# Bebra777228/PolGen-RVC

Measured on AMD Instinct MI355X. Metric: real-time-factor (audio-sec/wall-sec) per GPU, 30s@16kHz RMVPE->48kHz, higher is better.
Workload: dtype f32 (conv products as 3 fp16 MFMAs of a hi/lo split, fp32 accumulate; fp32 elsewhere)

## Files before the change

### polgen-rvc_amd/csrc/conv.h

```cpp
#pragma once
#include "common.h"

namespace rvcx {

enum Act { ACT_NONE = 0, ACT_LRELU = 1, ACT_RELU = 2, ACT_GELU = 3, ACT_TANH = 4, ACT_SIGMOID = 5 };
enum OutMode { OUT_NORMAL = 0, OUT_SHUF1D = 1, OUT_SHUF2D = 2, OUT_TRANSPOSED = 3 };
enum Acc2 { ACC2_NONE = 0, ACC2_SET = 1, ACC2_ADD = 2, ACC2_ADD_DIV = 3 };

struct ConvArgs {
  const float* x = nullptr;
  const float* w = nullptr;
  const void* w_h3 = nullptr;
  const void* x_split = nullptr;
  void* y_split = nullptr;
  const float* bias = nullptr;
  const float* res = nullptr;
  float* y = nullptr;
  float* y2 = nullptr;
  const int* lens_in = nullptr;
  const int* lens_out = nullptr;
  int B = 1;
  int Cin_g = 0, Cin_gp = 0, Cout_g = 0, Cout_gp = 0, groups = 1;
  int Tin = 0;
  int Nout = 0;
  int ksize = 1, kw = 1, rowpitch = 0, dil = 1, pad = 0, stride = 1;
  long x_bs = 0, y_bs = 0, res_bs = 0, y2_bs = 0;
  int x_cs = 0, y_cs = 0, res_cs = 0, y2_cs = 0;
  int pre_act = ACT_NONE;
  float pre_slope = 0.f;
  int act = ACT_NONE;
  float act_slope = 0.f;
  int out_mode = OUT_NORMAL;
  int sh_s = 1, sh_pad = 0, sh_cout = 0, sh_tout = 0;
  int wp_in = 0, wp_out = 0;
  int zero_wp = 0;
  int acc2_mode = ACC2_NONE;
  float acc2_div = 1.f;
  const float* nz_har = nullptr;
  const float* nz_w = nullptr;
  const float* nz_b = nullptr;
  const int* nz_lens = nullptr;
  int nz_k = 0, nz_stride = 1, nz_pad = 0, nz_wstride = 0;
  long nz_bs = 0;
  int nz_len = 0;
  float* part = nullptr;
  long part_cap = 0;
  long part_cap_item = 0;
  int ci_chunk = 0, kk_chunk = 0, wrow = 0, off_min = 0;
  int splitk = 1;
  long long* trace = nullptr;
  int stagger = 0;
  int stagger_blocks = 0;
  int* ovf = nullptr;
  int* ovf_layer = nullptr;
  int seq = 0;
  int dbg = 0;
};

inline int conv_tap_off(const ConvArgs& a, int kk) {
  return (kk / a.kw) * a.rowpitch + (kk % a.kw) * a.dil - a.pad;
}

struct PairArgs {
  const float* x = nullptr;
  float* y = nullptr;
  float* y2 = nullptr;
  const void* w1 = nullptr;
  const void* w2 = nullptr;
  const float* b1 = nullptr;
  const float* b2 = nullptr;
// ... 106 lines not shown
```

### polgen-rvc_amd/csrc/conv.hip

```cpp
#include "conv.h"
#include "conv_device.h"
#include "gemm.h"

#include <algorithm>
#include <cmath>

namespace rvcx {

template <int BM, int BN, int WR, int WC>
__global__ __launch_bounds__(256) void conv_mfma_kernel(const ConvArgs a) {
  constexpr int WM = BM / (32 * WR), WN = BN / (32 * WC);
  static_assert(WR * WC == 4 && WM >= 1 && WN >= 1, "bad tile");
  extern __shared__ float smem[];
  float* As = smem;
  float* Bs = smem + a.kk_chunk * a.ci_chunk * BM;

  const int tid = threadIdx.x, lane = tid & 63, wave = tid >> 6;
  const int wr = wave / WC, wc = wave % WC;
  const int i = lane & 31, h = lane >> 5;
  const int b = blockIdx.z;
  const int mt_per_g = (a.Cout_gp + BM - 1) / BM;
  const int g = blockIdx.y / mt_per_g, mt = blockIdx.y % mt_per_g;
  const int co0 = mt * BM;
  const int n0 = blockIdx.x * BN;
// ... 207 lines not shown
    return;
  }
  ProfRec rec;
  RVCX_HIP(hipEventCreate(&rec.a));
  RVCX_HIP(hipEventCreate(&rec.b));
  rec.tile = kBlock3Slot;
  rec.flops = flops;
  rec.cin = a.C; rec.cout = a.C; rec.k = 3; rec.nout = a.T; rec.stride = 135; rec.B = a.B;
  RVCX_HIP(hipEventRecord(rec.a, stream));
  launch_resblock3(a, stream);
  RVCX_HIP(hipEventRecord(rec.b, stream));
  g_prof.push_back(rec);
}

void conv_launch_gemm(const GemmArgs& a, double flops, hipStream_t stream) {
  if (!g_prof_on) {
    launch_gemm(a, stream);
    return;
  }
  ProfRec rec;
  RVCX_HIP(hipEventCreate(&rec.a));
  RVCX_HIP(hipEventCreate(&rec.b));
  rec.flops = flops;
  rec.cin = a.cin; rec.cout = a.cout; rec.k = 1; rec.nout = (int)a.rows; rec.stride = 1; rec.B = (int)(a.rows / a.T);
  RVCX_HIP(hipEventRecord(rec.a, stream));
  rec.tile = launch_gemm(a, stream);
  RVCX_HIP(hipEventRecord(rec.b, stream));
  g_prof.push_back(rec);
}

void launch_conv(ConvArgs a, hipStream_t stream) {
  RVCX_CHECK(a.Cin_gp % 2 == 0 && a.Cout_gp % 32 == 0, "conv: unpadded weights");
  RVCX_CHECK(a.Nout > 0 && a.B > 0, "conv: empty problem");
  if (g_prof_on) {
    ProfRec rec;
    RVCX_HIP(hipEventCreate(&rec.a));
    RVCX_HIP(hipEventCreate(&rec.b));
    rec.tile = 0;
    rec.flops = conv_flops(a);
    rec.cin = a.Cin_g * a.groups; rec.cout = a.Cout_g * a.groups; rec.k = a.ksize; rec.nout = a.Nout;
    rec.stride = a.stride; rec.B = a.B;
    RVCX_HIP(hipEventRecord(rec.a, stream));
    const int slot = launch_conv_fast(a, stream);
    if (slot >= 0) {
      rec.tile = slot;
      RVCX_HIP(hipEventRecord(rec.b, stream));
      g_prof.push_back(rec);
      return;
    }
    (void)hipEventDestroy(rec.a);
    (void)hipEventDestroy(rec.b);
  } else if (launch_conv_fast(a, stream) >= 0) {
    return;
  }
  int best = -1;
  double best_t = 1e300;
  ConvArgs best_a = a;
  for (int t = 0; t < kNumTiles; ++t) {
    ConvArgs c = a;
    if (!plan_lds(c, kTiles[t].bm, kTiles[t].bn)) continue;
    long mt = cdiv(a.Cout_gp, kTiles[t].bm), nt = cdiv(a.Nout, kTiles[t].bn);
    long blocks = mt * nt * a.groups;
    long rounds = (blocks + 511) / 512;
    double tm = (double)rounds * kTiles[t].bm * kTiles[t].bn / kTiles[t].eff;
    if (tm < best_t) {
      best_t = tm;
// ... 68 lines not shown
```

### polgen-rvc_amd/csrc/conv3_thin.hip

```cpp
#include <algorithm>
#include <cstdlib>
#include <mutex>

#include "conv.h"
#include "conv_device.h"
#include "h3_device.h"

namespace rvcx {

namespace {

constexpr int kTileN = 30;

__device__ __forceinline__ half8 shl1(half8 v) {
  uint4 u = __builtin_bit_cast(uint4, v);
#if defined(__HIP_DEVICE_COMPILE__)
  u.x = (unsigned)__builtin_amdgcn_update_dpp(0, (int)u.x, 0x130, 0xf, 0xf, false);
  u.y = (unsigned)__builtin_amdgcn_update_dpp(0, (int)u.y, 0x130, 0xf, 0xf, false);
  u.z = (unsigned)__builtin_amdgcn_update_dpp(0, (int)u.z, 0x130, 0xf, 0xf, false);
  u.w = (unsigned)__builtin_amdgcn_update_dpp(0, (int)u.w, 0x130, 0xf, 0xf, false);
#endif
  return __builtin_bit_cast(half8, u);
}

// ... 99 lines not shown
    }
    if (i < kTileN) {
      const int nn = p0 + i;
      if (a.y_split) store_tile_split(a, b, 0, nn, h, acc, len_out);
      else store_tile_fast(a, b, 4 * h, nn, acc, len_out);
    }
  }
  if (ovf) report_h3_overflow(a.ovf, a.ovf_layer, a.seq);
}

size_t lds_bytes(int cin) { return (size_t)(cin / 16) * 9 * 2 * 64 * 16; }

template <int CIN, bool XS>
void set_attr() {
  RVCX_HIP(hipFuncSetAttribute(reinterpret_cast<const void*>(conv3_thin_kernel<CIN, XS>),
                               hipFuncAttributeMaxDynamicSharedMemorySize, (int)lds_bytes(CIN)));
}

template <int CIN, bool XS>
void launch(const ConvArgs& a, dim3 grid, hipStream_t stream) {
  hipLaunchKernelGGL((conv3_thin_kernel<CIN, XS>), grid, dim3(256), lds_bytes(CIN), stream, a);
}

}

bool conv3_thin_ok(const ConvArgs& a) {
  static const bool on = !getenv("RVCX_CONV3_THIN") || atoi(getenv("RVCX_CONV3_THIN")) != 0;
  static const int min_n = getenv("RVCX_CONV3_THIN_MIN") ? atoi(getenv("RVCX_CONV3_THIN_MIN")) : 20000;
  if (!on || !a.w_h3 || !conv_h3_enabled() || g_conv_override.tile >= 0 || g_conv_override.splitk > 0) return false;
  if (a.groups != 1 || a.stride != 1 || a.dil != 1 || a.ksize != 9 || a.kw != 3 || a.rowpitch < 3 || a.pad != a.rowpitch + 1)
    return false;
  if (!(a.Cin_g == 16 || a.Cin_g == 32) || a.Cin_gp != a.Cin_g || a.Cout_g > 32 || a.Cout_gp > 32 || a.Cout_g < 1) return false;
  if (a.out_mode != OUT_NORMAL || a.act > ACT_RELU || a.pre_act != ACT_NONE || a.nz_har) return false;
  if (a.y_split && (a.Cout_g % 16 != 0 || a.acc2_mode != ACC2_NONE || a.res)) return false;
  if (!a.y_split && !a.y && a.acc2_mode == ACC2_NONE) return false;
  if ((long)a.Nout < min_n) return false;
  if ((long)a.Cin_g * a.x_cs * 4 >= kH3Oob || (long)a.Cout_g * a.y_cs * 4 >= kH3Oob) return false;
  return true;
}

void launch_conv3_thin(const ConvArgs& a, hipStream_t stream) {
  static std::mutex mu;
  static uint64_t done = 0;
  int dev = 0;
  RVCX_HIP(hipGetDevice(&dev));
  {
    std::lock_guard<std::mutex> g(mu);
    if (!((done >> (dev & 63)) & 1)) {
      set_attr<16, false>();
      set_attr<16, true>();
      set_attr<32, false>();
      set_attr<32, true>();
      done |= 1ull << (dev & 63);
    }
  }
  static const int ncu = [] {
    int d = 0, n = 256;
    if (hipGetDevice(&d) == hipSuccess) (void)hipDeviceGetAttribute(&n, hipDeviceAttributeMultiprocessorCount, d);
    return std::max(8, n);
  }();
  static const int per_cu_env = getenv("RVCX_CONV3_THIN_WGS") ? atoi(getenv("RVCX_CONV3_THIN_WGS")) : 0;
  const int per_cu = per_cu_env > 0 ? per_cu_env : (a.Cin_g == 16 ? 6 : 4);
  const int ntiles = cdiv(a.Nout, kTileN);
  const int per_xcd = cdiv(ntiles, 8), max_wg_x = std::max(1, ncu * per_cu / 8);
  const int rounds = cdiv(per_xcd, 4 * max_wg_x);
  const int wgs = 8 * std::max(1, cdiv(per_xcd, 4 * rounds));
// ... 14 lines not shown
```

### polgen-rvc_amd/csrc/conv_device.h

```cpp
#pragma once
#include "conv.h"

namespace rvcx {

typedef float f32x16 __attribute__((ext_vector_type(16)));

__device__ __forceinline__ void report_h3_overflow(int* ovf, int* layer, int seq) {
  if (ovf) atomicOr(ovf, kErrH3Overflow);
  if (layer) atomicMax(layer, 0x7fffffff - seq);
}

__device__ __forceinline__ float apply_act(float v, int act, float slope) {
  switch (act) {
    case ACT_LRELU: return v > 0.f ? v : v * slope;
    case ACT_RELU: return v > 0.f ? v : 0.f;
    case ACT_GELU: return 0.5f * v * (1.f + erff(v * 0.70710678118654752440f));
    case ACT_TANH: return tanhf(v);
    case ACT_SIGMOID: return 1.f / (1.f + __expf(-v));
    default: return v;
  }
}


__device__ __forceinline__ float noise_conv_at(const ConvArgs& a, int b, int c, int t) {
  const int nz_len = a.nz_lens ? a.nz_lens[b] : a.nz_len;
  const float* hb = a.nz_har + (long)b * a.nz_bs;
  const long p0 = (long)t * a.nz_stride - a.nz_pad;
  float n = 0.f;
  for (int j = 0; j < a.nz_k; ++j) {
    const long p = p0 + j;
    const float hvv = (p >= 0 && p < nz_len) ? hb[p] : 0.f;
    n = fmaf(a.nz_w[(long)j * a.nz_wstride + c], hvv, n);
  }
  return n + (a.nz_b ? a.nz_b[c] : 0.f);
}

__device__ __forceinline__ void store_elem(const ConvArgs& a, int b, int cg, int nn, float v, int len_out) {
  if (a.bias) v += a.bias[cg];
  v = apply_act(v, a.act, a.act_slope);
  if (a.out_mode == OUT_NORMAL) {
    if (a.res) v += a.res[(long)b * a.res_bs + (long)cg * a.res_cs + nn];
    if (nn >= len_out) v = 0.f;
    if (a.zero_wp > 0) {
      const int col = nn % a.zero_wp;
      if (col == 0 || col == a.zero_wp - 1) v = 0.f;
    }
    if (a.y) a.y[(long)b * a.y_bs + (long)cg * a.y_cs + nn] = v;
    if (a.acc2_mode != ACC2_NONE) {
      float* p2 = a.y2 + (long)b * a.y2_bs + (long)cg * a.y2_cs + nn;
      if (a.acc2_mode == ACC2_SET) *p2 = v;
      else if (a.acc2_mode == ACC2_ADD) *p2 = *p2 + v;
      else *p2 = (*p2 + v) / a.acc2_div;
    }
  } else if (a.out_mode == OUT_SHUF1D) {
    const int c = cg / a.sh_s, ph = cg - c * a.sh_s;
    const int t = nn * a.sh_s + ph - a.sh_pad;
    if (t >= 0 && t < a.sh_tout) {
      if (a.res) v += a.res[(long)b * a.res_bs + (long)c * a.res_cs + t];
      if (a.nz_har) v += noise_conv_at(a, b, c, t);
      if (t >= len_out) v = 0.f;
      a.y[(long)b * a.y_bs + (long)c * a.y_cs + t] = v;
    }
  } else if (a.out_mode == OUT_SHUF2D) {
    const int ph = cg / a.sh_cout, c = cg - ph * a.sh_cout;
    const int pa = ph >> 1, pb = ph & 1;
    const int irow = nn / a.wp_in, jj = nn - irow * a.wp_in;
    if (nn >= len_out) v = 0.f;
    if (jj != 0 && jj != a.wp_in - 1) {
      const long rowbase = (long)b * a.y_bs + (long)c * a.y_cs + (long)(2 * irow + pa) * a.wp_out;
      a.y[rowbase + 2 * (jj - 1) + pb + 1] = v;
      if (jj == 1 && pb == 0) a.y[rowbase] = 0.f;
      if (jj == a.wp_in - 2 && pb == 1) a.y[rowbase + a.wp_out - 1] = 0.f;
    }
  } else {
    if (a.res) v += a.res[(long)b * a.res_bs + (long)nn * a.res_cs + cg];
    if (nn >= len_out) v = 0.f;
    a.y[(long)b * a.y_bs + (long)nn * a.y_cs + cg] = v;
  }
}

__device__ __forceinline__ void store_tile(const ConvArgs& a, int b, int g, int co_base, int nn, const f32x16& t,
                                           int len_out) {
  if (nn >= a.Nout) return;
#pragma unroll
  for (int r = 0; r < 16; ++r) {
    const int co = co_base + (r & 3) + 8 * (r >> 2);
    if (co < a.Cout_g) store_elem(a, b, g * a.Cout_g + co, nn, t[r], len_out);
  }
}

__device__ __forceinline__ bool fast_epilogue_ok(const ConvArgs& a) {
  return a.out_mode == OUT_NORMAL && a.act <= ACT_RELU;
}

__device__ __forceinline__ void store_tile_fast(const ConvArgs& a, int b, int co_base, int nn, const f32x16& t,
                                                int len_out) {
  if (nn >= a.Nout) return;
  const float slope = a.act == ACT_NONE ? 1.f : (a.act == ACT_RELU ? 0.f : a.act_slope);
  bool live = nn < len_out;
  if (a.zero_wp > 0) {
    const int col = nn % a.zero_wp;
    live = live && col != 0 && col != a.zero_wp - 1;
  }
  float* yb = a.y ? a.y + (long)b * a.y_bs + nn : nullptr;
  const float* rb = a.res ? a.res + (long)b * a.res_bs + nn : nullptr;
  float* y2b = a.acc2_mode != ACC2_NONE ? a.y2 + (long)b * a.y2_bs + nn : nullptr;
#pragma unroll
  for (int r0 = 0; r0 < 16; r0 += 8) {
    float bv[8], rv[8];
#pragma unroll
    for (int q = 0; q < 8; ++q) {
      const int r = r0 + q;
      const int co = co_base + (r & 3) + 8 * (r >> 2);
      const int cc = co < a.Cout_g ? co : 0;
      bv[q] = a.bias ? a.bias[cc] : 0.f;
      rv[q] = rb ? rb[cc * a.res_cs] : 0.f;
    }
    if (y2b) {
      float pv[8];
#pragma unroll
      for (int q = 0; q < 8; ++q) {
        const int r = r0 + q;
        const int co = co_base + (r & 3) + 8 * (r >> 2);
        const int cc = co < a.Cout_g ? co : 0;
        pv[q] = a.acc2_mode != ACC2_SET ? y2b[cc * a.y2_cs] : 0.f;
// ... 71 lines not shown
```

### polgen-rvc_amd/csrc/conv_h3.hip

```cpp
#include <algorithm>
#include <cmath>
#include <cstdlib>

#include "conv.h"
#include "conv_device.h"
#include "h3_device.h"

#ifdef RVCX_ABLATION
#define H3_DBG(a, bit) ((a).dbg & (bit))
#else
#define H3_DBG(a, bit) 0
#endif

namespace rvcx {

template <int BM, int BN, int WR, int WC, int KKT, int HALO, int STRIDE, bool LIN, bool XS = false>
__global__ __launch_bounds__(256, ((LIN && BM * BN >= 8192) || BN >= 512) ? 2 : 3) void conv_h3_kernel(const ConvArgs a) {
  constexpr int WM = BM / (32 * WR), WN = BN / (32 * WC);
  constexpr int WROW = LIN ? BN : BN * STRIDE + HALO;
  constexpr int NBTILE = LIN ? KKT : 1;
  constexpr int A_ELEMS = KKT * 2 * 2 * BM;
  constexpr int NA = (A_ELEMS + 255) / 256;
  constexpr int B_TASKS = NBTILE * 2 * WROW;
  constexpr int NBT = (B_TASKS + 255) / 256;
  static_assert(WR * WC == 4, "bad tile");
  __shared__ uint4 As[A_ELEMS];
  __shared__ uint4 Bs[NBTILE * 2 * 2 * WROW];

  const int tid = threadIdx.x, lane = tid & 63, wave = tid >> 6;
  const int wr = wave / WC, wc = wave % WC;
  const int i = lane & 31, h = lane >> 5;
  const int bz = blockIdx.z / a.splitk, ks = blockIdx.z - bz * a.splitk;
  const int b = bz / a.groups, grp = bz - b * a.groups;
  const int co0 = blockIdx.y * BM;
  const int n0 = blockIdx.x * BN;
  const int len_in = a.lens_in ? a.lens_in[b] : a.Tin;
  const int in_base = n0 * STRIDE + a.off_min;
  const int wuse = LIN ? BN : BN * STRIDE + a.wrow;
  const int pre_act = a.pre_act;
  const float pre_slope = a.pre_slope;
  const int nchunk = a.Cin_gp / 16;
  constexpr bool xsplit = XS;
  static_assert(!XS || !LIN, "pre-split input: tap tiles only");
  const H3Rsrc xr = xsplit ? h3_rsrc(static_cast<const char*>(a.x_split) + (long)b * a.x_bs * 4, a.Cin_g * a.x_cs * 4)
                           : h3_rsrc(a.x + (long)b * a.x_bs + (long)grp * a.Cin_g * a.x_cs, a.Cin_g * a.x_cs * 4);
  const H3Rsrc wr_ = h3_rsrc(static_cast<const char*>(a.w_h3) + (long)grp * a.ksize * nchunk * 4 * a.Cout_gp * 16,
                             a.ksize * nchunk * 4 * a.Cout_gp * 16);

  f32x16 acc[WM][WN];
// ... 173 lines not shown
    }
    kk0 = kk1;
    chunk = chunk1;
  }

  if (ovf) report_h3_overflow(a.ovf, a.ovf_layer, a.seq);
  constexpr float inv = 1.f / kH3Scale;
#pragma unroll
  for (int m = 0; m < WM; ++m)
#pragma unroll
    for (int n = 0; n < WN; ++n)
#pragma unroll
      for (int r = 0; r < 16; ++r) acc[m][n][r] *= inv;

  const int co_w = co0 + wr * (WM * 32) + 4 * h, nn_w = n0 + wc * (WN * 32) + i;
  if (H3_DBG(a, 8)) return;
  if (a.splitk > 1) {
    float* pb = a.part + ((long)ks * a.B + b) * a.Cout_g * a.Nout;
#pragma unroll
    for (int m = 0; m < WM; ++m)
#pragma unroll
      for (int n = 0; n < WN; ++n) {
        const int nn = nn_w + n * 32;
        if (nn < a.Nout) {
#pragma unroll
          for (int r = 0; r < 16; ++r) {
            const int co = co_w + m * 32 + (r & 3) + 8 * (r >> 2);
            if (co < a.Cout_g) pb[(long)co * a.Nout + nn] = acc[m][n][r];
          }
        }
      }
    return;
  }
  if (a.y_split) {
    const int c_t = co0 + wr * (WM * 32);
#pragma unroll
    for (int m = 0; m < WM; ++m)
#pragma unroll
      for (int n = 0; n < WN; ++n) store_tile_split(a, b, c_t + m * 32, nn_w + n * 32, h, acc[m][n], len_out);
  } else if (fast_epilogue_ok(a) && a.groups == 1) {
#pragma unroll
    for (int m = 0; m < WM; ++m)
#pragma unroll
      for (int n = 0; n < WN; ++n) store_tile_fast(a, b, co_w + m * 32, nn_w + n * 32, acc[m][n], len_out);
  } else if (a.out_mode == OUT_SHUF1D) {
#pragma unroll
    for (int m = 0; m < WM; ++m)
#pragma unroll
      for (int n = 0; n < WN; ++n) store_tile_shuf1d(a, b, co_w + m * 32, nn_w + n * 32, acc[m][n], len_out);
  } else {
#pragma unroll
    for (int m = 0; m < WM; ++m)
#pragma unroll
      for (int n = 0; n < WN; ++n) store_tile(a, b, grp, co_w + m * 32, nn_w + n * 32, acc[m][n], len_out);
  }
}

namespace {
struct H3Cfg {
  int bm, bn, halo, stride;
  bool lin;
  float ovh;
  float eff;
  void (*kern)(const ConvArgs);
  void (*kern_xs)(const ConvArgs);
};
const H3Cfg kH3[] = {
    {32, 256, 64, 1, false, 18.f, 0.40f, conv_h3_kernel<32, 256, 1, 4, 4, 64, 1, false>, conv_h3_kernel<32, 256, 1, 4, 4, 64, 1, false, true>},
    {64, 128, 64, 1, false, 16.f, 0.45f, conv_h3_kernel<64, 128, 2, 2, 2, 64, 1, false>, conv_h3_kernel<64, 128, 2, 2, 2, 64, 1, false, true>},
    {64, 64, 64, 1, false, 16.f, 0.75f, conv_h3_kernel<64, 64, 2, 2, 4, 64, 1, false>, conv_h3_kernel<64, 64, 2, 2, 4, 64, 1, false, true>},
    {32, 128, 320, 1, false, 22.f, 1.00f, conv_h3_kernel<32, 128, 1, 4, 4, 320, 1, false>, conv_h3_kernel<32, 128, 1, 4, 4, 320, 1, false, true>},
    {64, 64, 320, 1, false, 20.f, 0.80f, conv_h3_kernel<64, 64, 2, 2, 4, 320, 1, false>, conv_h3_kernel<64, 64, 2, 2, 4, 320, 1, false, true>},
    {64, 128, 64, 2, false, 18.f, 0.50f, conv_h3_kernel<64, 128, 2, 2, 2, 64, 2, false>, conv_h3_kernel<64, 128, 2, 2, 2, 64, 2, false, true>},
    {64, 64, 64, 2, false, 16.f, 0.80f, conv_h3_kernel<64, 64, 2, 2, 4, 64, 2, false>, conv_h3_kernel<64, 64, 2, 2, 4, 64, 2, false, true>},
    {64, 64, 0, 1, true, 16.f, 0.95f, conv_h3_kernel<64, 64, 2, 2, 4, 0, 1, true>, nullptr},
    {128, 64, 0, 1, true, 18.f, 1.00f, conv_h3_kernel<128, 64, 4, 1, 2, 0, 1, true>, nullptr},
    {32, 256, 320, 1, false, 22.f, 1.10f, conv_h3_kernel<32, 256, 1, 4, 4, 320, 1, false>, conv_h3_kernel<32, 256, 1, 4, 4, 320, 1, false, true>},
    {32, 512, 320, 1, false, 22.f, 1.15f, conv_h3_kernel<32, 512, 1, 4, 4, 320, 1, false>, conv_h3_kernel<32, 512, 1, 4, 4, 320, 1, false, true>},
};
constexpr int kNumH3 = sizeof(kH3) / sizeof(kH3[0]);
constexpr int h3_slot(int t) { return t < 11 ? 39 + t : 28 + (t - 11); }
static_assert(kNumH3 <= 22, "conv_h3: out of profile slots");
}

thread_local bool g_force_fp32 = false;
thread_local bool g_gru_no_cluster = false;
thread_local int g_gru_drop_member = 0;

bool conv_h3_enabled() {
  static const int mode = getenv("RVCX_H3") ? atoi(getenv("RVCX_H3")) : 1;
  return mode != 0 && !g_force_fp32;
}

bool conv_h3_configured() {
  const bool saved = g_force_fp32;
  g_force_fp32 = false;
  const bool r = conv_h3_enabled();
  g_force_fp32 = saved;
  return r;
}

void conv_h3_describe(ConvProfile* p) {
  for (int t = 0; t < kNumH3; ++t) {
    const int s = h3_slot(t);
    p->bm[s] = kH3[t].bm;
    p->bn[s] = kH3[t].bn;
    p->halo[s] = 400000 + (kH3[t].lin ? 1 : (kH3[t].stride == 2 ? 2 : kH3[t].halo));
  }
}

bool conv_h3_split_ok(const ConvArgs& a) {
  if (!a.w_h3 || !conv_h3_enabled()) return false;
  if (a.groups != 1 || a.ksize == 1 || a.out_mode != OUT_NORMAL) return false;
  if (a.stride != 1 && !(a.stride == 2 && a.kw == a.ksize)) return false;
  if (a.Cin_g % 16 != 0 || a.Cout_g % 16 != 0 || a.Cin_g != a.Cin_gp) return false;
  {
    int lo = 1 << 30, hi = -(1 << 30);
    for (int kk = 0; kk < a.ksize; ++kk) {
      lo = std::min(lo, conv_tap_off(a, kk));
      hi = std::max(hi, conv_tap_off(a, kk));
    }
    if (hi - lo > 320) return false;
  }
  if ((long)a.Cin_gp * a.x_cs * 4 >= kH3Oob || (long)a.Cout_g * a.y_cs * 4 >= kH3Oob) return false;
  return true;
}

int launch_conv_h3(ConvArgs& a, int halo, int off_min, hipStream_t stream) {
  const bool split = a.x_split || a.y_split;
  RVCX_CHECK(!split || conv_h3_split_ok(a), "conv_h3: pre-split activations on a launch that cannot take them");
  if (!a.w_h3 || !conv_h3_enabled()) return -1;
  if (a.Cin_gp % 16 != 0 || (a.stride != 1 && !(a.stride == 2 && a.kw == a.ksize))) return -1;
  if (a.groups != 1 && (split || a.ksize == 1 || a.stride != 1 || a.out_mode != OUT_NORMAL || a.Cin_g != a.Cin_gp)) return -1;
  if ((long)a.Cin_gp * a.x_cs * 4 >= kH3Oob || (long)a.ksize * a.Cin_gp * a.Cout_gp * 4 >= kH3Oob) return -1;
  const bool lin = a.ksize == 1 && a.stride == 1;
  const int nchunk = a.Cin_gp / 16;
  const long cap_item = a.part_cap_item > 0 ? a.part_cap_item : a.part_cap;
  static const bool wide3x3 = getenv("RVCX_WIDE3X3") && atoi(getenv("RVCX_WIDE3X3")) != 0;
  auto select = [&](int Bsel, int forcedS, int* tile_out, int* s_out) {
    int best = -1, S = 1;
    double best_t = 1e300;
    for (int t = 0; t < kNumH3; ++t) {
      const H3Cfg& F = kH3[t];
      if (g_conv_override.tile >= 100 && g_conv_override.tile - 100 != t) continue;
      if (F.lin != lin || F.stride != a.stride) continue;
      if (a.x_split && !F.kern_xs) continue;
      if (!wide3x3 && g_conv_override.tile < 100 && F.halo == 320 && F.bn >= 256) continue;
      if (!lin && (halo > F.halo || (F.halo == 320 && halo <= 64))) continue;
      const long blocks = (long)cdiv(a.Cout_gp, F.bm) * cdiv(a.Nout, F.bn) * Bsel * a.groups;
      const double ksteps = (double)a.ksize * nchunk;
      for (int s = 1; s <= ((split || a.groups != 1) ? 1 : 8); s *= 2) {
        if (s > 1 && (!a.part || nchunk / s < 1 || ksteps / s < 8.0 || (long)s * a.Cout_g * a.Nout > cap_item ||
                      (long)s * a.B * a.Cout_g * a.Nout > a.part_cap))
          break;
        if (g_conv_override.splitk > 0 && g_conv_override.splitk != s) continue;
        if (forcedS > 0 && s != forcedS) continue;
        const double c = (double)blocks * s / 256.0;
        const double f = std::min(1.0, 0.45 + 0.55 * (std::max(c, 1.0) - 1.0) / 3.0);
        double us = std::ceil(c) * (F.bm / 32) * (F.bn / 32) * (ksteps / s + F.ovh) / (39.0 * F.eff * f);
        if (s > 1) us += 3.0 + (double)(s + 1) * Bsel * a.Cout_g * a.Nout * 4.0 / 3e6;
        if (us < best_t) {
          best_t = us;
          best = t;
          S = s;
        }
      }
    }
    *tile_out = best;
    *s_out = S;
  };
  int best = -1, S = 1;
  select(1, 0, &best, &S);
  static const int tile2_mask = getenv("RVCX_TILE2_MASK") ? atoi(getenv("RVCX_TILE2_MASK")) : 255;
  const int cls = (a.out_mode != OUT_NORMAL) ? 8 : (lin ? 2 : (halo > 64 ? 1 : 4));
  int cls2 = cls;
  if (a.x_split || a.y_split) cls2 |= 16;
  const bool tile_for_batch = (tile2_mask & cls) && (!(cls2 & 16) || (tile2_mask & 16));
  if (best >= 0 && a.B > 1 && tile_for_batch) {
    int b2 = -1, s2 = 1;
    select(a.B, S, &b2, &s2);
    if (b2 >= 0 && s2 == S) best = b2;
  }
  if (best < 0) return -1;
  const H3Cfg& F = kH3[best];
  a.off_min = off_min;
  a.wrow = halo;
  a.splitk = S;
  {
    static int dbg = -1;
    if (dbg < 0) dbg = getenv("RVCX_CONV_DBG") ? atoi(getenv("RVCX_CONV_DBG")) : 0;
    a.dbg = dbg;
  }
  dim3 grid(cdiv(a.Nout, F.bn), cdiv(a.Cout_gp, F.bm), a.B * a.groups * S);
  {
    static const bool log = getenv("RVCX_CONV_LOG") != nullptr;
    if (log)
      fprintf(stderr, "h3 tile %d (%dx%d halo %d) S %d grid %u %u %u B %d Cin %d Cout %d k %d Nout %d xs %d ys %d\n", best,
              F.bm, F.bn, F.halo, S, grid.x, grid.y, grid.z, a.B, a.Cin_g, a.Cout_g, a.ksize, a.Nout, a.x_split != nullptr,
              a.y_split != nullptr);
  }
  hipLaunchKernelGGL(a.x_split ? F.kern_xs : F.kern, grid, dim3(256), 0, stream, a);
  if (S > 1) launch_splitk_finish(a, stream);
  RVCX_HIP(hipGetLastError());
  return h3_slot(best);
}

}
```

### polgen-rvc_amd/csrc/models.h

```cpp
#pragma once
#include <functional>

#include "../../include/rvcx.h"
#include "ctx.h"
#include "layers.h"

namespace rvcx {

struct SynthModel {
  std::shared_ptr<WeightRegion> region = std::make_shared<WeightRegion>();
  rvcx_synth_cfg cfg{};
  int upp = 1;
  int dec_rf_frames = 0;
  ConvW emb_phone;
  const float* emb_pitch = nullptr;
  struct EncLayer {
    ConvW qkv, o, ffn1, ffn2;
    AttFlag att;
    const float *rel_k = nullptr, *rel_v = nullptr;
    const float *g1 = nullptr, *b1 = nullptr, *g2 = nullptr, *b2 = nullptr;
  };
  std::vector<EncLayer> enc;
  ConvW proj;
  struct Flow {
    ConvW pre, post, cond, in_l[3], rs_l[3];
  };
  Flow flows[4];
  ConvW conv_pre, cond, conv_post;
  const float* lin_wb = nullptr;
  struct Stage {
    ConvT1dW up;
    ConvW noise;
    int noise_stride = 1, noise_pad = 0;
    ConvW noise_dense;
    int noise_dense_cin = 0;
    int ch = 0;
    ConvW c1[4][3], c2[4][3];
  };
  std::vector<Stage> stages;
  const float* emb_g = nullptr;
};

std::unique_ptr<SynthModel> synth_load(Ctx& c, const rvcx_synth_cfg& cfg, const TensorTable& t);

struct SynthIO {
  int B = 1, T = 0;
  const int* lens_host = nullptr;
  const float* phone_ct = nullptr;
  const int* pitch = nullptr;
  const float* pitchf = nullptr;
  const int* sid_host = nullptr;
  const float* z_noise = nullptr;
  const float* src_noise = nullptr;
  float* out = nullptr;
  int dec_skip = 0;
  int skip_head = 0;
  float* stats_out = nullptr;
  float* z_out = nullptr;
  hipEvent_t ev_decoder = nullptr;
};
size_t synth_arena_bytes(const SynthModel& m, int B, int T);
void synth_forward(Ctx& c, const SynthModel& m, const SynthIO& io, hipEvent_t* stage_ev );

struct RmvpeModel {
  std::shared_ptr<WeightRegion> region = std::make_shared<WeightRegion>();
  rvcx_rmvpe_cfg cfg{};
  ConvW stft;
  ConvW melfb;
  const float* bn0 = nullptr;
  struct Block {
    ConvW c1, c2, sc;
    bool has_sc = false;
    int cin = 0, cout = 0;
  };
// ... 130 lines not shown
```

### polgen-rvc_amd/csrc/synth.hip

```cpp
#include <algorithm>
#include <cmath>
#include <cstdlib>

#include "models.h"
#include "ops.h"

namespace rvcx {

std::vector<float> wn_weight(const TensorTable& t, const std::string& p, int dim) {
  if (t.has(p + ".weight")) return t.f32(p + ".weight");
  std::string gn = p + ".parametrizations.weight.original0", vn = p + ".parametrizations.weight.original1";
  if (!t.has(gn)) {
    gn = p + ".weight_g";
    vn = p + ".weight_v";
  }
  std::vector<float> g = t.f32(gn), v = t.f32(vn);
  const auto shp = t.shape(vn);
  RVCX_CHECK(shp.size() == 3, "weight-norm tensor must be 3-D: " + p);
  const int64_t d0 = shp[0], d1 = shp[1], d2 = shp[2];
  std::vector<float> w(v.size());
  if (dim == 0) {
    RVCX_CHECK((int64_t)g.size() == d0, "weight_g shape: " + p);
    for (int64_t a = 0; a < d0; ++a) {
      double ss = 0.0;
// ... 143 lines not shown
size_t synth_arena_bytes(const SynthModel& m, int B, int T) {
  const auto& cf = m.cfg;
  size_t enc = (size_t)B * T * (size_t)(cf.input_dim + 8 * cf.hidden_channels + 2 * cf.filter_channels +
                                        4 * cf.inter_channels + 64 + (8 * 98 + 2 * 96 + 8) * cf.n_heads);
  size_t dec = (size_t)B * T * m.upp * 5;
  size_t mx = 0, sum = (size_t)B * T * cf.up_initial_channel;
  long tt = T;
  for (size_t i = 0; i < m.stages.size(); ++i) {
    tt *= cf.up_rates[i];
    const size_t n = (size_t)B * tt * m.stages[i].ch;
    mx = std::max(mx, n);
    sum += n + 1024;
  }
  return (enc + dec + 2 * sum + 9 * mx) * sizeof(float) + ((size_t)64 << 20);
}

namespace {

struct Timer3 {
  Ctx& c;
  hipEvent_t* e;
  Timer3(Ctx& cc, hipEvent_t* ev) : c(cc), e(ev) {}
  void mark(int i) {
    if (e) RVCX_HIP(hipEventRecord(e[i], c.stream));
  }
};

int* upload_ints(Ctx& c, const std::vector<int>& v) {
  int* d = c.arena.alloc<int>(v.size());
  RVCX_HIP(hipMemcpyAsync(d, v.data(), v.size() * sizeof(int), hipMemcpyHostToDevice, c.stream));
  return d;
}

}

void synth_forward(Ctx& c, const SynthModel& m, const SynthIO& io, hipEvent_t* stage_ev) {
  const auto& cf = m.cfg;
  const int B = io.B, T = io.T, hid = cf.hidden_channels, inter = cf.inter_channels, filt = cf.filter_channels;
  const int heads = cf.n_heads, kc = hid / heads, half = inter / 2, gin = cf.gin_channels;
  hipStream_t s = c.stream;
  Arena& A = c.arena;
  Timer3 tm(c, stage_ev);
  tm.mark(0);
  const int head = io.skip_head, Tk = T - head;
  RVCX_CHECK(head >= 0 && Tk > 0, "synth: skip_head outside [0, T)");
  if (head > 0) {
    RVCX_CHECK(io.dec_skip == 0, "synth: dec_skip and skip_head exclude each other");
    if (io.lens_host)
      for (int b = 0; b < B; ++b) RVCX_CHECK(io.lens_host[b] == T, "synth: skip_head needs equal lengths (every item T frames)");
  }

  bool ragged = false;
  if (io.lens_host)
    for (int b = 0; b < B; ++b) ragged |= io.lens_host[b] != T;
  std::vector<const int*> lens_stage(m.stages.size() + 2, nullptr);
  const int* lens = nullptr;
  if (ragged) {
    std::vector<int> l(io.lens_host, io.lens_host + B);
    lens = upload_ints(c, l);
    lens_stage[0] = lens;
    for (size_t i = 0; i < m.stages.size(); ++i) {
      for (auto& x : l) x *= cf.up_rates[i];
      lens_stage[i + 1] = upload_ints(c, l);
    }
  }
  std::vector<int> sidv(io.sid_host, io.sid_host + B);
// ... 78 lines not shown
    a.lens_out = lens;
    conv_set_res(a, x, hid, T);
    c.conv(a);
    launch_layernorm_c(tmp, L.g1, L.b1, x, B, hid, T, 1e-5f, nullptr, s);
    const int k = L.ffn1.k, pl = (k - 1) / 2;
    a = conv1d_args(L.ffn1, x, hbuf, B, T, T, 1, 1, pl);
    a.act = ACT_RELU;
    a.lens_in = lens;
    a.lens_out = lens;
    c.conv(a);
    a = conv1d_args(L.ffn2, hbuf, tmp, B, T, T, 1, 1, pl);
    a.lens_in = lens;
    a.lens_out = lens;
    conv_set_res(a, x, hid, T);
    c.conv(a);
    launch_layernorm_c(tmp, L.g2, L.b2, x, B, hid, T, 1e-5f, nullptr, s);
  }
  float* stats = io.stats_out ? io.stats_out : A.alloc<float>((size_t)B * 2 * inter * T);
  {
    launch_mask(x, B, hid, T, lens, s);
    ConvArgs a = conv1d_args(m.proj, x, stats, B, T, T);
    a.lens_out = lens;
    c.conv(a);
  }
  tm.mark(1);

  float* z = A.alloc<float>((size_t)B * inter * T);
  float* z2 = A.alloc<float>((size_t)B * inter * T);
  launch_sample_z(stats, io.z_noise, z, B, inter, T, lens, s);
  if (head > 0) {
    launch_copy_strided(z + head, z2, B * inter, Tk, T, Tk, s);
    std::swap(z, z2);
  }
  float* g = A.alloc<float>((size_t)B * gin);
  for (int b = 0; b < B; ++b)
    RVCX_HIP(hipMemcpyAsync(g + (size_t)b * gin, m.emb_g + (size_t)sidv[b] * gin, gin * sizeof(float),
                            hipMemcpyDeviceToDevice, s));
  {
    float* h = att;
    float* xin = qkv;
    float* acts = tmp;
    float* rs = hbuf;
    RVCX_CHECK(filt >= 2 * hid, "buffer reuse assumes filter_channels >= 2*hidden");
    float* wout = A.alloc<float>((size_t)B * hid * T);
    float* mbuf = A.alloc<float>((size_t)B * half * T);
    float* gc = A.alloc<float>((size_t)B * 6 * hid);
    for (int f = 3; f >= 0; --f) {
      const auto& F = m.flows[f];
      launch_flip_channels(z, z2, B, inter, Tk, s);
      std::swap(z, z2);
      ConvArgs a = conv1d_args(F.pre, z, h, B, Tk, Tk);
      a.x_bs = (long)inter * Tk;
      a.lens_out = lens;
      c.conv(a);
      a = conv1d_args(F.cond, g, gc, B, 1, 1);
      c.conv(a);
      for (int i = 0; i < 3; ++i) {
        a = conv1d_args(F.in_l[i], h, xin, B, Tk, Tk, 1, 1, (F.in_l[i].k - 1) / 2);
        a.lens_in = lens;
        a.lens_out = lens;
        c.conv(a);
        launch_wn_gate(xin, gc, i * 2 * hid, 6 * hid, acts, B, hid, Tk, s);
        a = conv1d_args(F.rs_l[i], acts, rs, B, Tk, Tk);
        a.lens_out = lens;
        c.conv(a);
        launch_wn_res_skip(h, wout, rs, B, hid, Tk, i == 2, i == 0, lens, s);
      }
      a = conv1d_args(F.post, wout, mbuf, B, Tk, Tk);
      a.lens_out = lens;
      c.conv(a);
      launch_coupling_sub(z, mbuf, B, half, Tk, lens, s);
    }
  }
  if (io.z_out)
    RVCX_HIP(hipMemcpyAsync(io.z_out, z, (size_t)B * inter * Tk * sizeof(float), hipMemcpyDeviceToDevice, s));
  tm.mark(2);
  if (io.ev_decoder) RVCX_HIP(hipEventRecord(io.ev_decoder, s));

  if (!c.serial) RVCX_HIP(hipStreamWaitEvent(s, c.ev_src[1], 0));
  static const int dec_batch_env = getenv("RVCX_DEC_BATCH") ? std::max(1, atoi(getenv("RVCX_DEC_BATCH"))) : 8;
  bool equal_lens = true;
  if (io.lens_host)
    for (int b = 1; b < B; ++b) equal_lens &= io.lens_host[b] == io.lens_host[0];
  const int dec_batch = equal_lens ? dec_batch_env : 1;
  const int C0 = cf.up_initial_channel;
  const size_t dec_mark = A.mark();
  for (int b0 = 0; b0 < B; b0 += dec_batch) {
    const int db = std::min(dec_batch, B - b0);
    A.reset(dec_mark);
    const bool own = io.lens_host != nullptr && (db == 1 || equal_lens);
    const int Tfull = own ? io.lens_host[b0] - head : Tk;
    RVCX_CHECK(Tfull > 0 && Tfull <= Tk, "synth: item length outside (0, T]");
    const int skip = (io.dec_skip > 0 && (own || !lens) && Tfull - 2 * io.dec_skip > 2 * m.dec_rf_frames) ? io.dec_skip : 0;
    const int Td = Tfull - 2 * skip;
    float* cur = A.alloc<float>((size_t)db * C0 * Td);
    {
      ConvArgs a = conv1d_args(m.conv_pre, z + (size_t)b0 * inter * Tk + skip, cur, db, Td, Td, 1, 1, 3);
      a.x_bs = (long)inter * Tk;
      a.x_cs = Tk;
      a.lens_in = (lens && !own) ? lens + b0 : nullptr;
      c.conv(a);
      float* gcond = A.alloc<float>((size_t)db * C0);
      a = conv1d_args(m.cond, g + (size_t)b0 * gin, gcond, db, 1, 1);
      c.conv(a);
      launch_add_channel_bias(cur, gcond, db, C0, Td, s);
    }
    long Tin = Td, Tin_c = Tk, off = skip;
    for (size_t i = 0; i < m.stages.size(); ++i) {
      const auto& S = m.stages[i];
      const long Tout = Tin * cf.up_rates[i], Tout_c = Tin_c * cf.up_rates[i];
      off *= cf.up_rates[i];
      const size_t n = (size_t)db * S.ch * Tout;
      float* xs = A.alloc<float>(n);
      const size_t stage_mark = A.mark();
      float* xu = A.alloc<float>(n);
      const int nk = cf.n_resblocks;
      float* xcb[4];
      float* xtb[4];
      for (int j = 0; j < nk; ++j) {
        xcb[j] = A.alloc<float>(n);
        xtb[j] = A.alloc<float>(n);
      }
      const int* lin = (lens_stage[i] && !own) ? lens_stage[i] + b0 : nullptr;
      const int* lout = (lens_stage[i + 1] && !own) ? lens_stage[i + 1] + b0 : nullptr;
      ConvArgs a = convT1d_args(S.up, cur, xu, db, (int)Tin, (int)Tout);
      a.pre_act = ACT_LRELU;
      a.pre_slope = 0.1f;
      a.lens_in = lin;
      a.lens_out = lout;
      if (nz_fused[i]) {
        a.nz_har = har + (size_t)b0 * Tupp + (size_t)skip * m.upp;
        a.nz_bs = Tupp;
        a.nz_w = S.noise.w;
        a.nz_wstride = S.noise.cin_gp * S.noise.cout_gp;
        a.nz_b = S.noise.bias;
        a.nz_k = S.noise.k;
        a.nz_stride = S.noise_stride;
        a.nz_pad = S.noise_pad;
// ... 150 lines not shown
```

Baseline: 1242.

## Fold flow residual/skip, coupling and speaker-conditioning adds into conv epilogues

Adds folded epilogue modes to the conv store path: add a per-channel vector (add2), subtract from the residual (res_sub), and split output channels across two destinations (co_split). These replace the separate wn_res_skip, coupling_sub and add_channel_bias kernels in the flow and decoder-pre stages. Speaker-conditioning conv outputs are cached per speaker id and recomputed only when the weight region changes, which removes the per-forward cond convs and embedding copies. The trade-off is a new FOLD template variant available on only some h3 tiles, so tile selection can be forced onto a different tile, plus more branching in the generic store path.

```diff
diff --git a/polgen-rvc_amd/csrc/conv.h b/polgen-rvc_amd/csrc/conv.h
--- a/polgen-rvc_amd/csrc/conv.h
+++ b/polgen-rvc_amd/csrc/conv.h
@@ -36,6 +36,12 @@
   int zero_wp = 0;
   int acc2_mode = ACC2_NONE;
   float acc2_div = 1.f;
+  const float* add2 = nullptr;
+  long add2_bs = 0;
+  int res_sub = 0;
+  int co_split = 0;
+  float* y_hi = nullptr;
+  const float* res_hi = nullptr;
   const float* nz_har = nullptr;
   const float* nz_w = nullptr;
   const float* nz_b = nullptr;
diff --git a/polgen-rvc_amd/csrc/conv.hip b/polgen-rvc_amd/csrc/conv.hip
--- a/polgen-rvc_amd/csrc/conv.hip
+++ b/polgen-rvc_amd/csrc/conv.hip
@@ -263,6 +263,12 @@
 void launch_conv(ConvArgs a, hipStream_t stream) {
   RVCX_CHECK(a.Cin_gp % 2 == 0 && a.Cout_gp % 32 == 0, "conv: unpadded weights");
   RVCX_CHECK(a.Nout > 0 && a.B > 0, "conv: empty problem");
+  if (a.add2 || a.res_sub || a.co_split > 0) {
+    RVCX_CHECK(a.out_mode == OUT_NORMAL && a.groups == 1 && a.y && !a.y_split && a.acc2_mode == ACC2_NONE && a.zero_wp == 0,
+               "conv: add2 / res_sub / co_split need a plain OUT_NORMAL store");
+    RVCX_CHECK(!a.res_sub || a.res, "conv: res_sub without a residual");
+    RVCX_CHECK(a.co_split <= 0 || (a.y_hi && a.co_split < a.Cout_g), "conv: co_split needs y_hi and a row inside the layer");
+  }
   if (g_prof_on) {
     ProfRec rec;
     RVCX_HIP(hipEventCreate(&rec.a));
diff --git a/polgen-rvc_amd/csrc/conv3_thin.hip b/polgen-rvc_amd/csrc/conv3_thin.hip
--- a/polgen-rvc_amd/csrc/conv3_thin.hip
+++ b/polgen-rvc_amd/csrc/conv3_thin.hip
@@ -155,6 +155,7 @@
     return false;
   if (!(a.Cin_g == 16 || a.Cin_g == 32) || a.Cin_gp != a.Cin_g || a.Cout_g > 32 || a.Cout_gp > 32 || a.Cout_g < 1) return false;
   if (a.out_mode != OUT_NORMAL || a.act > ACT_RELU || a.pre_act != ACT_NONE || a.nz_har) return false;
+  if (a.add2 || a.res_sub || a.co_split > 0) return false;
   if (a.y_split && (a.Cout_g % 16 != 0 || a.acc2_mode != ACC2_NONE || a.res)) return false;
   if (!a.y_split && !a.y && a.acc2_mode == ACC2_NONE) return false;
   if ((long)a.Nout < min_n) return false;
diff --git a/polgen-rvc_amd/csrc/conv_device.h b/polgen-rvc_amd/csrc/conv_device.h
--- a/polgen-rvc_amd/csrc/conv_device.h
+++ b/polgen-rvc_amd/csrc/conv_device.h
@@ -35,7 +35,27 @@
   return n + (a.nz_b ? a.nz_b[c] : 0.f);
 }
 
+__device__ __forceinline__ void store_elem_fold(const ConvArgs& a, int b, int cg, int nn, float v, int len_out) {
+  if (a.bias) v += a.bias[cg];
+  v = apply_act(v, a.act, a.act_slope);
+  const bool hi = a.co_split > 0 && cg >= a.co_split;
+  const float* res = hi ? a.res_hi : a.res;
+  float* y = hi ? a.y_hi : a.y;
+  const int cr = hi ? cg - a.co_split : cg;
+  if (res) {
+    const float rv = res[(long)b * a.res_bs + (long)cr * a.res_cs + nn];
+    v = a.res_sub ? rv - v : v + rv;
+  }
+  if (a.add2) v += a.add2[(long)b * a.add2_bs + cg];
+  if (nn >= len_out) v = 0.f;
+  y[(long)b * a.y_bs + (long)cr * a.y_cs + nn] = v;
+}
+
 __device__ __forceinline__ void store_elem(const ConvArgs& a, int b, int cg, int nn, float v, int len_out) {
+  if (a.add2 || a.res_sub || a.co_split > 0) {
+    store_elem_fold(a, b, cg, nn, v, len_out);
+    return;
+  }
   if (a.bias) v += a.bias[cg];
   v = apply_act(v, a.act, a.act_slope);
   if (a.out_mode == OUT_NORMAL) {
@@ -89,8 +109,57 @@
   }
 }
 
+__device__ __forceinline__ bool conv_fold_form(const ConvArgs& a) { return a.add2 || a.res_sub || a.co_split > 0; }
 __device__ __forceinline__ bool fast_epilogue_ok(const ConvArgs& a) {
-  return a.out_mode == OUT_NORMAL && a.act <= ACT_RELU;
+  return a.out_mode == OUT_NORMAL && a.act <= ACT_RELU && !conv_fold_form(a);
+}
+
+__device__ __forceinline__ void store_tile_fold(const ConvArgs& a, int b, int co_base, int nn, const f32x16& t,
+                                                int len_out) {
+  if (nn >= a.Nout) return;
+  const int lo = co_base & ~31;
+  const bool hi = a.co_split > 0 && lo >= a.co_split;
+  if (a.co_split > 0 && !hi && lo + 32 > a.co_split) {
+#pragma unroll
+    for (int r = 0; r < 16; ++r) {
+      const int co = co_base + (r & 3) + 8 * (r >> 2);
+      if (co < a.Cout_g) store_elem(a, b, co, nn, t[r], len_out);
+    }
+    return;
+  }
+  const float slope = a.act == ACT_NONE ? 1.f : (a.act == ACT_RELU ? 0.f : a.act_slope);
+  const bool live = nn < len_out;
+  const int cs = hi ? a.co_split : 0;
+  float* yd = hi ? a.y_hi : a.y;
+  const float* rd = hi ? a.res_hi : a.res;
+  float* yb = yd + (long)b * a.y_bs + nn;
+  const float* rb = rd ? rd + (long)b * a.res_bs + nn : nullptr;
+  const float* gb = a.add2 ? a.add2 + (long)b * a.add2_bs : nullptr;
+#pragma unroll
+  for (int r0 = 0; r0 < 16; r0 += 8) {
+    float bv[8], rv[8], gv[8];
+#pragma unroll
+    for (int q = 0; q < 8; ++q) {
+      const int r = r0 + q;
+      const int co = co_base + (r & 3) + 8 * (r >> 2);
+      const int cc = co < a.Cout_g ? co : cs;
+      bv[q] = a.bias ? a.bias[cc] : 0.f;
+      rv[q] = rb ? rb[(long)(cc - cs) * a.res_cs] : 0.f;
+      gv[q] = gb ? gb[cc] : 0.f;
+    }
+#pragma unroll
+    for (int q = 0; q < 8; ++q) {
+      const int r = r0 + q;
+      const int co = co_base + (r & 3) + 8 * (r >> 2);
+      if (co < a.Cout_g) {
+        float v = t[r] + bv[q];
+        v = fmaxf(v, v * slope);
+        if (rb) v = a.res_sub ? rv[q] - v : v + rv[q];
+        if (gb) v += gv[q];
+        yb[(long)(co - cs) * a.y_cs] = live ? v : 0.f;
+      }
+    }
+  }
 }
 
 __device__ __forceinline__ void store_tile_fast(const ConvArgs& a, int b, int co_base, int nn, const f32x16& t,
diff --git a/polgen-rvc_amd/csrc/conv_h3.hip b/polgen-rvc_amd/csrc/conv_h3.hip
--- a/polgen-rvc_amd/csrc/conv_h3.hip
+++ b/polgen-rvc_amd/csrc/conv_h3.hip
@@ -14,7 +14,7 @@
 
 namespace rvcx {
 
-template <int BM, int BN, int WR, int WC, int KKT, int HALO, int STRIDE, bool LIN, bool XS = false>
+template <int BM, int BN, int WR, int WC, int KKT, int HALO, int STRIDE, bool LIN, bool XS = false, bool FOLD = false>
 __global__ __launch_bounds__(256, ((LIN && BM * BN >= 8192) || BN >= 512) ? 2 : 3) void conv_h3_kernel(const ConvArgs a) {
   constexpr int WM = BM / (32 * WR), WN = BN / (32 * WC);
   constexpr int WROW = LIN ? BN : BN * STRIDE + HALO;
@@ -254,6 +254,13 @@
       }
     return;
   }
+  if constexpr (FOLD) {
+#pragma unroll
+    for (int m = 0; m < WM; ++m)
+#pragma unroll
+      for (int n = 0; n < WN; ++n) store_tile_fold(a, b, co_w + m * 32, nn_w + n * 32, acc[m][n], len_out);
+    return;
+  }
   if (a.y_split) {
     const int c_t = co0 + wr * (WM * 32);
 #pragma unroll
@@ -286,16 +293,18 @@
   float eff;
   void (*kern)(const ConvArgs);
   void (*kern_xs)(const ConvArgs);
+  void (*kern_fold)(const ConvArgs) = nullptr;
 };
 const H3Cfg kH3[] = {
     {32, 256, 64, 1, false, 18.f, 0.40f, conv_h3_kernel<32, 256, 1, 4, 4, 64, 1, false>, conv_h3_kernel<32, 256, 1, 4, 4, 64, 1, false, true>},
     {64, 128, 64, 1, false, 16.f, 0.45f, conv_h3_kernel<64, 128, 2, 2, 2, 64, 1, false>, conv_h3_kernel<64, 128, 2, 2, 2, 64, 1, false, true>},
-    {64, 64, 64, 1, false, 16.f, 0.75f, conv_h3_kernel<64, 64, 2, 2, 4, 64, 1, false>, conv_h3_kernel<64, 64, 2, 2, 4, 64, 1, false, true>},
+    {64, 64, 64, 1, false, 16.f, 0.75f, conv_h3_kernel<64, 64, 2, 2, 4, 64, 1, false>, conv_h3_kernel<64, 64, 2, 2, 4, 64, 1, false, true>,
+     conv_h3_kernel<64, 64, 2, 2, 4, 64, 1, false, false, true>},
     {32, 128, 320, 1, false, 22.f, 1.00f, conv_h3_kernel<32, 128, 1, 4, 4, 320, 1, false>, conv_h3_kernel<32, 128, 1, 4, 4, 320, 1, false, true>},
     {64, 64, 320, 1, false, 20.f, 0.80f, conv_h3_kernel<64, 64, 2, 2, 4, 320, 1, false>, conv_h3_kernel<64, 64, 2, 2, 4, 320, 1, false, true>},
     {64, 128, 64, 2, false, 18.f, 0.50f, conv_h3_kernel<64, 128, 2, 2, 2, 64, 2, false>, conv_h3_kernel<64, 128, 2, 2, 2, 64, 2, false, true>},
     {64, 64, 64, 2, false, 16.f, 0.80f, conv_h3_kernel<64, 64, 2, 2, 4, 64, 2, false>, conv_h3_kernel<64, 64, 2, 2, 4, 64, 2, false, true>},
-    {64, 64, 0, 1, true, 16.f, 0.95f, conv_h3_kernel<64, 64, 2, 2, 4, 0, 1, true>, nullptr},
+    {64, 64, 0, 1, true, 16.f, 0.95f, conv_h3_kernel<64, 64, 2, 2, 4, 0, 1, true>, nullptr, conv_h3_kernel<64, 64, 2, 2, 4, 0, 1, true, false, true>},
     {128, 64, 0, 1, true, 18.f, 1.00f, conv_h3_kernel<128, 64, 4, 1, 2, 0, 1, true>, nullptr},
     {32, 256, 320, 1, false, 22.f, 1.10f, conv_h3_kernel<32, 256, 1, 4, 4, 320, 1, false>, conv_h3_kernel<32, 256, 1, 4, 4, 320, 1, false, true>},
     {32, 512, 320, 1, false, 22.f, 1.15f, conv_h3_kernel<32, 512, 1, 4, 4, 320, 1, false>, conv_h3_kernel<32, 512, 1, 4, 4, 320, 1, false, true>},
@@ -359,14 +368,17 @@
   const int nchunk = a.Cin_gp / 16;
   const long cap_item = a.part_cap_item > 0 ? a.part_cap_item : a.part_cap;
   static const bool wide3x3 = getenv("RVCX_WIDE3X3") && atoi(getenv("RVCX_WIDE3X3")) != 0;
-  auto select = [&](int Bsel, int forcedS, int* tile_out, int* s_out) {
+  const bool fold = a.add2 || a.res_sub || a.co_split > 0;
+  RVCX_CHECK(!(fold && split), "conv_h3: the folded epilogue forms do not take pre-split activations");
+  auto select = [&](int Bsel, int forcedS, int* tile_out, int* s_out, bool fold_tiles = false) {
     int best = -1, S = 1;
     double best_t = 1e300;
     for (int t = 0; t < kNumH3; ++t) {
       const H3Cfg& F = kH3[t];
-      if (g_conv_override.tile >= 100 && g_conv_override.tile - 100 != t) continue;
+      if (!fold_tiles && g_conv_override.tile >= 100 && g_conv_override.tile - 100 != t) continue;
       if (F.lin != lin || F.stride != a.stride) continue;
       if (a.x_split && !F.kern_xs) continue;
+      if (fold_tiles && !F.kern_fold) continue;
       if (!wide3x3 && g_conv_override.tile < 100 && F.halo == 320 && F.bn >= 256) continue;
       if (!lin && (halo > F.halo || (F.halo == 320 && halo <= 64))) continue;
       const long blocks = (long)cdiv(a.Cout_gp, F.bm) * cdiv(a.Nout, F.bn) * Bsel * a.groups;
@@ -404,6 +416,12 @@
     if (b2 >= 0 && s2 == S) best = b2;
   }
   if (best < 0) return -1;
+  if (fold && !kH3[best].kern_fold) {
+    int b2 = -1, s2 = 1;
+    select(a.B, S, &b2, &s2, true);
+    RVCX_CHECK(b2 >= 0 && s2 == S, "conv_h3: no tile with the folded epilogue forms for this launch");
+    best = b2;
+  }
   const H3Cfg& F = kH3[best];
   a.off_min = off_min;
   a.wrow = halo;
@@ -421,7 +439,7 @@
               F.bm, F.bn, F.halo, S, grid.x, grid.y, grid.z, a.B, a.Cin_g, a.Cout_g, a.ksize, a.Nout, a.x_split != nullptr,
               a.y_split != nullptr);
   }
-  hipLaunchKernelGGL(a.x_split ? F.kern_xs : F.kern, grid, dim3(256), 0, stream, a);
+  hipLaunchKernelGGL(fold ? F.kern_fold : (a.x_split ? F.kern_xs : F.kern), grid, dim3(256), 0, stream, a);
   if (S > 1) launch_splitk_finish(a, stream);
   RVCX_HIP(hipGetLastError());
   return h3_slot(best);
diff --git a/polgen-rvc_amd/csrc/models.h b/polgen-rvc_amd/csrc/models.h
--- a/polgen-rvc_amd/csrc/models.h
+++ b/polgen-rvc_amd/csrc/models.h
@@ -1,5 +1,6 @@
 #pragma once
 #include <functional>
+#include <map>
 
 #include "../../include/rvcx.h"
 #include "ctx.h"
@@ -39,7 +40,23 @@
   };
   std::vector<Stage> stages;
   const float* emb_g = nullptr;
-};
+  struct CondCache {
+    struct Row {
+      float* d = nullptr;
+      bool valid = false;
+    };
+    std::map<int, Row> rows;
+    int dropped = 0;
+    ~CondCache() {
+      for (auto& kv : rows) (void)hipFree(kv.second.d);
+    }
+  };
+  mutable CondCache cond_cache;
+  size_t cond_row_floats() const { return (size_t)4 * 6 * cfg.hidden_channels + cfg.up_initial_channel; }
+};
+
+enum FoldItem { FOLD_COND = 1, FOLD_RES_SKIP = 3, FOLD_COUPLING = 4 };
+bool fold_on(FoldItem item);
 
 std::unique_ptr<SynthModel> synth_load(Ctx& c, const rvcx_synth_cfg& cfg, const TensorTable& t);
 
diff --git a/polgen-rvc_amd/csrc/synth.hip b/polgen-rvc_amd/csrc/synth.hip
--- a/polgen-rvc_amd/csrc/synth.hip
+++ b/polgen-rvc_amd/csrc/synth.hip
@@ -199,6 +199,32 @@
   return d;
 }
 
+const float* cond_row(Ctx& c, const SynthModel& m, int sid) {
+  auto& cc = m.cond_cache;
+  if (cc.dropped != m.region->dropped()) {
+    for (auto& kv : cc.rows) kv.second.valid = false;
+    cc.dropped = m.region->dropped();
+  }
+  auto& row = cc.rows[sid];
+  if (!row.d) RVCX_HIP(hipMalloc(&row.d, m.cond_row_floats() * sizeof(float)));
+  if (row.valid) return row.d;
+  const int hid = m.cfg.hidden_channels, gin = m.cfg.gin_channels;
+  const float* g = m.emb_g + (size_t)sid * gin;
+  for (int f = 0; f < 4; ++f) c.conv(conv1d_args(m.flows[f].cond, g, row.d + (size_t)f * 6 * hid, 1, 1, 1));
+  c.conv(conv1d_args(m.cond, g, row.d + (size_t)4 * 6 * hid, 1, 1, 1));
+  row.valid = true;
+  return row.d;
+}
+
+}
+
+bool fold_on(FoldItem item) {
+  static const int mask = [] {
+    const char* e = getenv("RVCX_FOLD");
+    const long v = e ? strtol(e, nullptr, 0) : 1;
+    return v == 1 ? ~0 : (int)v;
+  }();
+  return (mask >> item) & 1;
 }
 
 void synth_forward(Ctx& c, const SynthModel& m, const SynthIO& io, hipEvent_t* stage_ev) {
@@ -343,10 +369,30 @@
     launch_copy_strided(z + head, z2, B * inter, Tk, T, Tk, s);
     std::swap(z, z2);
   }
-  float* g = A.alloc<float>((size_t)B * gin);
-  for (int b = 0; b < B; ++b)
-    RVCX_HIP(hipMemcpyAsync(g + (size_t)b * gin, m.emb_g + (size_t)sidv[b] * gin, gin * sizeof(float),
-                            hipMemcpyDeviceToDevice, s));
+  const bool fold_cond = fold_on(FOLD_COND) && !g_force_fp32;
+  const bool fold_rs = fold_on(FOLD_RES_SKIP), fold_cpl = fold_on(FOLD_COUPLING);
+  const float* condp = nullptr;
+  long cond_bs = 0;
+  float* g = nullptr;
+  if (fold_cond) {
+    bool one = true;
+    for (int b = 1; b < B; ++b) one &= sidv[b] == sidv[0];
+    if (one) {
+      condp = cond_row(c, m, sidv[0]);
+    } else {
+      const size_t R = m.cond_row_floats();
+      float* rows = A.alloc<float>((size_t)B * R);
+      for (int b = 0; b < B; ++b)
+        RVCX_HIP(hipMemcpyAsync(rows + (size_t)b * R, cond_row(c, m, sidv[b]), R * sizeof(float), hipMemcpyDeviceToDevice, s));
+      condp = rows;
+      cond_bs = (long)R;
+    }
+  } else {
+    g = A.alloc<float>((size_t)B * gin);
+    for (int b = 0; b < B; ++b)
+      RVCX_HIP(hipMemcpyAsync(g + (size_t)b * gin, m.emb_g + (size_t)sidv[b] * gin, gin * sizeof(float),
+                              hipMemcpyDeviceToDevice, s));
+  }
   {
     float* h = att;
     float* xin = qkv;
@@ -364,23 +410,53 @@
       a.x_bs = (long)inter * Tk;
       a.lens_out = lens;
       c.conv(a);
-      a = conv1d_args(F.cond, g, gc, B, 1, 1);
-      c.conv(a);
+      const float* gf = gc;
+      long gf_bs = 6 * hid;
+      if (fold_cond) {
+        gf = condp + (size_t)f * 6 * hid;
+        gf_bs = cond_bs;
+      } else {
+        a = conv1d_args(F.cond, g, gc, B, 1, 1);
+        c.conv(a);
+      }
       for (int i = 0; i < 3; ++i) {
         a = conv1d_args(F.in_l[i], h, xin, B, Tk, Tk, 1, 1, (F.in_l[i].k - 1) / 2);
         a.lens_in = lens;
         a.lens_out = lens;
         c.conv(a);
-        launch_wn_gate(xin, gc, i * 2 * hid, 6 * hid, acts, B, hid, Tk, s);
+        launch_wn_gate(xin, gf, i * 2 * hid, (int)gf_bs, acts, B, hid, Tk, s);
         a = conv1d_args(F.rs_l[i], acts, rs, B, Tk, Tk);
         a.lens_out = lens;
-        c.conv(a);
-        launch_wn_res_skip(h, wout, rs, B, hid, Tk, i == 2, i == 0, lens, s);
+        if (fold_rs) {
+          a.y_bs = (long)hid * Tk;
+          if (i == 2) {
+            a.y = wout;
+            conv_set_res(a, wout, hid, Tk);
+          } else {
+            a.y = h;
+            conv_set_res(a, h, hid, Tk);
+            a.co_split = hid;
+            a.y_hi = wout;
+            a.res_hi = i == 0 ? nullptr : wout;
+          }
+          c.conv(a);
+        } else {
+          c.conv(a);
+          launch_wn_res_skip(h, wout, rs, B, hid, Tk, i == 2, i == 0, lens, s);
+        }
       }
       a = conv1d_args(F.post, wout, mbuf, B, Tk, Tk);
       a.lens_out = lens;
-      c.conv(a);
-      launch_coupling_sub(z, mbuf, B, half, Tk, lens, s);
+      if (fold_cpl) {
+        a.y = z + (size_t)half * Tk;
+        a.y_bs = (long)inter * Tk;
+        conv_set_res(a, a.y, inter, Tk);
+        a.res_sub = 1;
+        c.conv(a);
+      } else {
+        c.conv(a);
+        launch_coupling_sub(z, mbuf, B, half, Tk, lens, s);
+      }
     }
   }
   if (io.z_out)
@@ -410,11 +486,17 @@
       a.x_bs = (long)inter * Tk;
       a.x_cs = Tk;
       a.lens_in = (lens && !own) ? lens + b0 : nullptr;
-      c.conv(a);
-      float* gcond = A.alloc<float>((size_t)db * C0);
-      a = conv1d_args(m.cond, g + (size_t)b0 * gin, gcond, db, 1, 1);
-      c.conv(a);
-      launch_add_channel_bias(cur, gcond, db, C0, Td, s);
+      if (fold_cond) {
+        a.add2 = condp + (size_t)b0 * cond_bs + (size_t)4 * 6 * hid;
+        a.add2_bs = cond_bs;
+        c.conv(a);
+      } else {
+        c.conv(a);
+        float* gcond = A.alloc<float>((size_t)db * C0);
+        a = conv1d_args(m.cond, g + (size_t)b0 * gin, gcond, db, 1, 1);
+        c.conv(a);
+        launch_add_channel_bias(cur, gcond, db, C0, Td, s);
+      }
     }
     long Tin = Td, Tin_c = Tk, off = skip;
     for (size_t i = 0; i < m.stages.size(); ++i) {
```

Result: no change. 1247 (median of 5 runs) (+0.4%).
